# DrQuestion/monica

Hardware: AMD Instinct MI355X
Metric: reads/sec classified (higher is better)
Workload: dtype u32/u64 integer; int16 pairs in the alignment kernels (int32 / int8 in the long-call and literal ones); float32 islands: overlap ratio, MAPQ

## Files before the change

### monica_amd/csrc/k_fill.hip

```cpp
#include "device.h"

namespace mnc {

constexpr int FILL_NEG = -(1 << 28);
constexpr int FILL_WIN = 16;
constexpr int FILL_MIN_BAND = 8;
constexpr int FILL_CIG_MAX = 384;
constexpr size_t FILL_P_SLOT = (size_t)(2 * FILL_MAX_LEN + FILL_WIN) * 64;

__device__ __forceinline__ void fill_order()
{
	__builtin_amdgcn_fence(__ATOMIC_SEQ_CST, "wavefront");
	asm volatile("" ::: "memory");
}
__device__ __forceinline__ void fill_order_mem()
{
	__builtin_amdgcn_fence(__ATOMIC_SEQ_CST, "workgroup");
	asm volatile("" ::: "memory");
}

__device__ __forceinline__ int fill_nt4(uint8_t c)
{
	switch (c) {
	case 'A': case 'a': return 0;
// ... 287 lines not shown
				}
			}
			if (max_zdrop > (B.zdrop_inv < B.zdrop ? B.zdrop_inv : B.zdrop)) to_fb = true;
		}
		const bool s_next = __shfl((int)to_next, lead) != 0, s_fb = __shfl((int)to_fb, lead) != 0;
		const int s_nc = __shfl(n_c, lead);
		if (has && (s_next || s_fb)) {
			if (leader) {
				const bool literal = s_fb || next_list == fb_list;
				if (literal && (B.segs[si].flag & SEG_NEEDS_BIG_WS)) { const unsigned long long k = atomicAdd(&B.dp_ctr[56], 1ULL); B.bigfb_list[k] = (int32_t)si; }
				else if (literal) { const unsigned long long k = atomicAdd(&B.dp_ctr[ctr_fb], 1ULL); fb_list[k] = (int32_t)si; }
				else { const unsigned long long k = atomicAdd(&B.dp_ctr[ctr_next], 1ULL); next_list[k] = (int32_t)si; }
			}
		} else if (has) {
			unsigned long long off = 0;
			if (leader) off = atomicAdd(&B.dp_ctr[1], (unsigned long long)s_nc);
			off = (unsigned long long)__shfl((long long)off, lead);
			int wrote = s_nc;
			if ((long long)(off + s_nc) > B.cig_seg_cap) {
				if (leader) atomicMax(&B.dp_ctr[4], 2ULL);
				wrote = 0;
			} else for (int k = L; k < s_nc; k += LANES) B.cig_seg[off + k] = s_cg[sg][s_nc - 1 - k];
			if (leader) {
				Seg *o = B.segs + si;
				o->n_cigar = wrote, o->zdropped = 0, o->zdrop_code = 0;
				o->max = 0, o->max_t = -1, o->max_q = -1, o->score = S, o->reach_end = 0, o->mqe_t = -1;
				o->cig_off = (int64_t)off;
			}
		}
		fill_order_mem();
	}
}

typedef short pk_s16 __attribute__((ext_vector_type(2)));
typedef unsigned short pk_u16 __attribute__((ext_vector_type(2)));
__device__ __forceinline__ uint32_t pk_adds(uint32_t x, uint32_t y) { return __builtin_bit_cast(uint32_t, __builtin_elementwise_add_sat(__builtin_bit_cast(pk_s16, x), __builtin_bit_cast(pk_s16, y))); }
__device__ __forceinline__ uint32_t pk_subs(uint32_t x, uint32_t y) { return __builtin_bit_cast(uint32_t, __builtin_elementwise_sub_sat(__builtin_bit_cast(pk_s16, x), __builtin_bit_cast(pk_s16, y))); }
__device__ __forceinline__ uint32_t pk_maxs(uint32_t x, uint32_t y) { return __builtin_bit_cast(uint32_t, __builtin_elementwise_max(__builtin_bit_cast(pk_s16, x), __builtin_bit_cast(pk_s16, y))); }
__device__ __forceinline__ uint32_t pk_subsu(uint32_t x, uint32_t y) { return __builtin_bit_cast(uint32_t, __builtin_elementwise_sub_sat(__builtin_bit_cast(pk_u16, x), __builtin_bit_cast(pk_u16, y))); }
__device__ __forceinline__ uint32_t pk_madu(uint32_t x, uint32_t y, uint32_t z) { return __builtin_bit_cast(uint32_t, (pk_u16)(__builtin_bit_cast(pk_u16, x) * __builtin_bit_cast(pk_u16, y) + __builtin_bit_cast(pk_u16, z))); }
__device__ __forceinline__ uint32_t pk_rep(int v) { return ((uint32_t)v & 0xffffu) * 0x10001u; }
__device__ __forceinline__ uint32_t pk_bfi(uint32_t mask, uint32_t x, uint32_t y) { return (x & mask) | (y & ~mask); }

constexpr uint32_t PK_NEG = 0x80008000u;
__device__ __forceinline__ uint32_t fillp_opened(uint32_t x)
{
	const uint32_t d = (x & 1u) ^ 1u, c = (x >> 1 & 1u) ^ d, b = (x >> 2 & 1u) ^ 1u ^ c ^ d, a = (x >> 3 & 1u) ^ b ^ c ^ d;
	return a << 3 | b << 2 | c << 1 | d;
}
constexpr uint32_t PK_TAG_H = 0x000f000fu, PK_TAG_E = 0x00070007u, PK_TAG_F = 0x00030003u, PK_TAG_E2 = 0x00010001u;
struct PkConst { uint32_t kmatch, kmis, q8, q28, e8, e28, de28, dstep; int bias; };

__host__ __device__ __forceinline__ bool fillp_bias(int cells, int a, int bmis_abs, int q, int e, int q2, int e2, int &bias)
{
	const int hi = a * FILL_MAX_LEN, lo = -(bmis_abs * FILL_MAX_LEN + fill_gap(2 * cells + 2, q, e, q2, e2) + (q + e > q2 + e2 ? q + e : q2 + e2));
	bias = -(hi + lo) / 2;
	return hi + bias < 2040 && lo + bias > -2040;
}
__host__ __device__ __forceinline__ bool fillp_drifts(int bmis_abs, int e, int e2) { return bmis_abs == 2 * e && e >= e2; }
__host__ __device__ __forceinline__ bool fillp_bias_drift(int a, int q, int e, int q2, int e2, int &bias)
{
	const int hi = (a + 2 * e) * FILL_MAX_LEN, lo = -(q + e + q2 + e2 + 64);
	bias = -(hi + lo) / 2;
	return hi + bias < 2040 && lo + bias > -2040;
}

template <int K> __device__ __forceinline__ uint32_t fillp_next_q(uint32_t Q2, uint32_t w) { return __builtin_amdgcn_perm(Q2, w, 0x05040c00u + K); }
template <int K> __device__ __forceinline__ uint32_t fillp_next_t(uint32_t T2, uint32_t w) { return __builtin_amdgcn_perm(w, T2, 0x0c040302u + K * 0x10000u); }

#ifndef MNC_FILLP_FRAME2
#define MNC_FILLP_FRAME2 1
#endif
template <int LANES, int ODD, bool EDGE, bool CAPTURE = true, bool DRIFT = false, int KB = -1>
__device__ __forceinline__ void fillp_step(const PkConst &K, const int r, const int L, const int rows_m1, const uint8_t *st, const uint8_t *sq,
                                           const int q, const int e, const int q2, const int e2,
                                           int &t_lo, int &tn, int &jn, uint32_t &T2, uint32_t &Q2, uint32_t &Hs,
                                           uint32_t &E, uint32_t &E2, uint32_t &F, uint32_t &F2, uint32_t &Sc,
                                           uint32_t &nb1, uint32_t &nb2, uint32_t &acc, const uint32_t wq = 0, const uint32_t wt = 0)
{
	constexpr int SHR = LANES == 16 ? 0x111 : 0x138, SHL = LANES == 16 ? 0x101 : 0x130;
	constexpr bool SEG_EDGES = LANES != 16 && LANES != 64;
	uint32_t vE, vE2, vF, vF2;
	if (!ODD) {
		nb1 = (uint32_t)__builtin_amdgcn_update_dpp((int)nb1, (int)E, SHR, 0xf, 0xf, false);
		nb2 = (uint32_t)__builtin_amdgcn_update_dpp((int)nb2, (int)E2, SHR, 0xf, 0xf, false);
		if (SEG_EDGES && L == 0) nb1 = nb2 = PK_NEG;
		vE = __builtin_amdgcn_alignbit(E, nb1, 16), vE2 = __builtin_amdgcn_alignbit(E2, nb2, 16);
		vF = F, vF2 = F2;
		if constexpr (KB >= 0) Q2 = fillp_next_q<KB & 3>(Q2, wq);
		else Q2 = __builtin_amdgcn_perm(Q2, (uint32_t)sq[jn], 0x05040100u), ++jn;
	} else {
		nb1 = (uint32_t)__builtin_amdgcn_update_dpp((int)nb1, (int)F, SHL, 0xf, 0xf, false);
		nb2 = (uint32_t)__builtin_amdgcn_update_dpp((int)nb2, (int)F2, SHL, 0xf, 0xf, false);
		if (SEG_EDGES && L == LANES - 1) nb1 = nb2 = PK_NEG;
		vF = __builtin_amdgcn_alignbit(nb1, F, 16), vF2 = __builtin_amdgcn_alignbit(nb2, F2, 16);
		vE = E, vE2 = E2;
		if constexpr (KB >= 0) T2 = fillp_next_t<KB & 3>(T2, wt);
		else T2 = __builtin_amdgcn_perm((uint32_t)st[tn], T2, 0x05040302u), ++tn;
		if (EDGE) ++t_lo;
	}
	uint32_t hd = Hs;
	if (EDGE) {
		const int hb = -fill_gap(r + 1, q, e, q2, e2) + K.bias + (DRIFT ? e * r : 0);
		const uint32_t h0 = pk_rep(((r == 0 ? 0 : -fill_gap(r, q, e, q2, e2)) + K.bias + (DRIFT ? e * (r - 2) : 0)) << 4) | PK_TAG_H;
		const uint32_t g1 = pk_rep((hb - q - e) << 4), g2 = pk_rep((hb - q2 - e2) << 4);
		const uint32_t mt = t_lo == 0 ? 0x0000ffffu : t_lo == -1 ? 0xffff0000u : 0u;
		const uint32_t mj = t_lo == r ? 0x0000ffffu : t_lo == r - 1 ? 0xffff0000u : 0u;
		hd = pk_bfi(mt | mj, h0, hd);
		vE = pk_bfi(mt, g1 | PK_TAG_E, vE), vE2 = pk_bfi(mt, g2 | PK_TAG_E2, vE2);
		vF = pk_bfi(mj, g1 | PK_TAG_F, vF), vF2 = pk_bfi(mj, g2, vF2);
	}
	uint32_t z;
	if (DRIFT) z = pk_madu(pk_subsu(0x00010001u, T2 ^ Q2), K.kmatch, hd);
	else z = pk_adds(hd, pk_madu(pk_subsu(0x00010001u, T2 ^ Q2), K.kmatch, K.kmis));
	uint32_t o2sub = K.q28;
	constexpr bool FRAME2 = DRIFT && MNC_FILLP_FRAME2 && LANES <= 32;
	if (FRAME2) {
		const uint32_t Dr = (uint32_t)r * K.dstep;
		z = pk_maxs(z, vE), z = pk_maxs(z, vF), z = pk_maxs(z, pk_adds(pk_maxs(vE2, vF2), Dr));
		o2sub = K.q28 + Dr;
	} else z = pk_maxs(z, vE), z = pk_maxs(z, vF), z = pk_maxs(z, vE2), z = pk_maxs(z, vF2);
	const uint32_t zt = z | PK_TAG_H;
	const uint32_t o1 = pk_subs(zt, K.q8), o2 = pk_subs(zt, o2sub);
	const uint32_t mE = pk_maxs(vE, o1), mF = pk_maxs(vF, o1), mE2 = pk_maxs(vE2, o2), mF2 = pk_maxs(vF2, o2);
	if (FRAME2) {
		E = mE & 0xfff7fff7u, F = mF & 0xfff3fff3u, E2 = mE2 & 0xfff1fff1u, F2 = mF2 & 0xfff0fff0u;
	} else if (DRIFT) {
		E = mE & 0xfff7fff7u, F = mF & 0xfff3fff3u;
		E2 = pk_adds(mE2, K.de28) & 0xfff1fff1u, F2 = pk_adds(mF2, K.de28) & 0xfff0fff0u;
	} else {
		E = pk_subs(mE, K.e8) & 0xfff7fff7u;
		F = pk_subs(mF, K.e8) & 0xfff3fff3u;
		E2 = pk_subs(mE2, K.e28) & 0xfff1fff1u;
		F2 = pk_subs(mF2, K.e28) & 0xfff0fff0u;
	}
	const uint32_t x3 = (uint32_t)__builtin_amdgcn_bitop3_b32((int)mE, (int)mF, (int)mE2, 0x96);
	const uint32_t d = pk_bfi(0x000f000fu, z, (x3 ^ mF2) << 4);
	acc = ODD ? __builtin_amdgcn_perm(d, acc, 0x06040200u) : d;
	if (CAPTURE) Sc = r == rows_m1 ? zt : Sc;
	Hs = zt;
}

constexpr int FILLP_G = 16, FILLP_G_MAX = 21;
template <int LANES> struct FillpShape {
	static constexpr int SEGS = 64 / LANES;
	static constexpr int G = SEGS == 3 ? 21 : FILLP_G;
};
constexpr int FILLP_BLOCKS = (2 * FILL_MAX_LEN + 15) / 16 + 1;
constexpr size_t FILLP_PASS_BYTES = (size_t)FILLP_BLOCKS * 64 * 32;
constexpr size_t FILLP_SLOT = FILLP_G_MAX * FILLP_PASS_BYTES;

#ifndef MNC_FILLP_WAVES
#define MNC_FILLP_WAVES 4
#endif
template <int LANES, bool DRIFT>
__global__ __launch_bounds__(64, MNC_FILLP_WAVES) void mnc_dp_fillp(Batch B, const int32_t *list, int ctr_n, int ctr_q, int32_t *next_list, int ctr_next,
                                                   int32_t *fb_list, int ctr_fb, uint8_t *p_all, uint32_t *cig_all)
{
	constexpr int SEGS = FillpShape<LANES>::SEGS, G_MAX = FillpShape<LANES>::G, W = 2 * LANES;
	constexpr int PAD = ((2 * W + 8) & ~7) - 1, SEQ = (FILL_MAX_LEN + 1 + 4 * W + 32 + 7) & ~7;
	static_assert(SEGS * G_MAX <= 64, "one walk per lane");
	constexpr int V = DRIFT ? 1 : 0;
	__shared__ __align__(16) uint8_t s_t[SEGS][SEQ], s_q[SEGS][SEQ];
	__shared__ __align__(16) uint8_t s_chunk[64][32];
	__shared__ int32_t s_n[64], s_m[64], s_kmin[64], s_S[64], s_si[64], s_state[64];
	__shared__ int32_t s_item[64];
	const int lane = threadIdx.x;
	const bool live = lane < SEGS * LANES;
	const int sg = live ? lane / LANES : 0, L = live ? lane % LANES : 0, lead = sg * LANES;
	const bool leader = live && L == 0;
	const int a = B.sc_a, bmis = -B.sc_b, q = B.gap_q, e = B.gap_e, q2 = B.gap_q2, e2 = B.gap_e2;
	PkConst K;
	K.kmatch = pk_rep((DRIFT ? a + 2 * e : a - bmis) << 4), K.kmis = pk_rep(bmis << 4), K.q8 = pk_rep(q << 4), K.q28 = pk_rep(q2 << 4), K.e8 = pk_rep(e << 4), K.e28 = pk_rep(e2 << 4);
	K.de28 = pk_rep((e - e2) << 4), K.dstep = K.de28;
	const bool fits = DRIFT ? fillp_bias_drift(a, q, e, q2, e2, K.bias) : fillp_bias(W, a, -bmis > B.sc_ambi ? -bmis : B.sc_ambi, q, e, q2, e2, K.bias);
	uint8_t *p_wave = p_all + (size_t)blockIdx.x * FILLP_SLOT;
	uint32_t *cg = cig_all + ((size_t)blockIdx.x * 64 + lane) * FILL_CIG_MAX;
	const unsigned long long n_items = B.dp_ctr[ctr_n];
	const unsigned long long segmask = LANES == 64 ? ~0ULL : ((1ULL << (LANES & 63)) - 1) << lead;
	const int thr = B.zdrop_inv < B.zdrop ? B.zdrop_inv : B.zdrop;
	int g_eff = (int)((n_items + (unsigned long long)gridDim.x * SEGS - 1) / ((unsigned long long)gridDim.x * SEGS));
	if (g_eff > G_MAX && g_eff < 2 * G_MAX) g_eff = (g_eff + 1) / 2;
	g_eff = g_eff < 1 ? 1 : g_eff > G_MAX ? G_MAX : g_eff;
	for (;;) {
		unsigned long long q0 = 0;
		if (lane == 0) q0 = atomicAdd(&B.dp_ctr[ctr_q], (unsigned long long)(g_eff * SEGS));
		q0 = (unsigned long long)__shfl((long long)q0, 0);
		if (q0 >= n_items) break;
		s_state[lane] = 0;
		{
			int my_si = -1, my_rows = INT32_MAX;
			if (lane < g_eff * SEGS && q0 + lane < n_items) {
				my_si = list[q0 + lane];
				const Seg *gs = B.segs + my_si;
				my_rows = gs->tlen + gs->qlen;
			}
			int rank = 0;
			for (int j = 0; j < 64; ++j) {
				const int rj = __shfl(my_rows, j);
				rank += (rj < my_rows || (rj == my_rows && j < lane)) ? 1 : 0;
			}
			s_item[rank] = my_si;
		}
		fill_order();
		for (int u = 0; u < g_eff; ++u) {
			if (q0 + (unsigned long long)u * SEGS >= n_items) break;
			const long long si = live ? s_item[u * SEGS + sg] : -1;
			const bool has = si >= 0;
			struct { int32_t tlen, qlen, ts, qs, read, rid, rev; } g = { 0, 0, 0, 0, 0, 0, 0 };
			if (has) {
				const Seg *gs = B.segs + si;
				g.tlen = gs->tlen, g.qlen = gs->qlen, g.ts = gs->ts, g.qs = gs->qs, g.read = gs->read, g.rid = gs->rid, g.rev = gs->rev;
			}
			const int n = g.tlen, m = g.qlen;
			int b, kmin, kmax;
			fill_band(n, m, W, b, kmin, kmax);
			bool ok = has && fits && n >= 1 && m >= 1 && n <= FILL_MAX_LEN && m <= FILL_MAX_LEN && b >= FILL_MIN_BAND;
			bool ambiguous = false;
			if (ok) {
				const uint8_t *read = B.bases + B.offsets[g.read];
				const int rlen = (int)(B.offsets[g.read + 1] - B.offsets[g.read]);
				const int64_t coff = B.seq_off[g.rid] + g.ts;
				const bool acgt = !B.ambig[g.read];
				const int64_t roff = B.offsets[g.read];
				if (V) {
					const uint32_t sh = (uint32_t)(coff & 7) * 4;
#pragma unroll 1
					for (int i = 8 * L; i < n; i += 8 * LANES) {
						const bool more = sh != 0 && i + 8 - (int)(coff & 7) < n;
						const uint32_t a0 = B.seq4[((coff + i) >> 3)], a1 = more ? B.seq4[((coff + i) >> 3) + 1] : 0u;
						const uint32_t v = sh ? __builtin_amdgcn_alignbit(a1, a0, sh) : a0;
						ambiguous |= (v & 0xccccccccu & (n - i < 8 ? (1u << (4 * (n - i))) - 1u : ~0u)) != 0;
						uint2 w;
						w.x = v & 0xffffu, w.x = (w.x | w.x << 8) & 0x00ff00ffu, w.x = (w.x | w.x << 4) & 0x03030303u;
						w.y = v >> 16, w.y = (w.y | w.y << 8) & 0x00ff00ffu, w.y = (w.y | w.y << 4) & 0x03030303u;
						*reinterpret_cast<uint2*>(&s_t[sg][PAD + 1 + i]) = w;
					}
					if (acgt) {
#pragma unroll 1
						for (int i = 16 * L; i < m; i += 16 * LANES) {
							const uint32_t f = fill_qcodes16(B, roff, rlen, g.rev, g.qs + i);
							uint32_t x[4];
#pragma unroll
							for (int k = 0; k < 4; ++k) {
								const uint32_t b8 = f >> (8 * k) & 0xffu;
								x[k] = (b8 | b8 << 12) & 0x000f000fu, x[k] = (x[k] | x[k] << 6) & 0x03030303u;
							}
							*reinterpret_cast<uint2*>(&s_q[sg][PAD + 1 + i]) = make_uint2(x[0], x[1]);
							*reinterpret_cast<uint2*>(&s_q[sg][PAD + 1 + i + 8]) = make_uint2(x[2], x[3]);
						}
					} else {
#pragma unroll 1
						for (int i = L; i < m; i += LANES) {
							const int c = fill_qcode(B, false, roff, read, rlen, g.rev, g.qs + i);
							ambiguous |= c > 3;
							s_q[sg][PAD + 1 + i] = (uint8_t)(c & 3);
						}
					}
					if (L == 0) s_t[sg][PAD] = 4, s_q[sg][PAD] = 5;
				} else {
#pragma unroll 1
					for (int i = L; i < n; i += LANES) {
						const int64_t o = coff + i;
						const uint32_t c = B.seq4[o >> 3] >> ((o & 7) * 4) & 15u;
						ambiguous |= c > 3;
						s_t[sg][PAD + i] = (uint8_t)(c & 3);
					}
#pragma unroll 1
					for (int i = L; i < m; i += LANES) {
						const int c = fill_qcode(B, acgt, roff, read, rlen, g.rev, g.qs + i);
						ambiguous |= c > 3;
						s_q[sg][PAD + i] = (uint8_t)(c & 3);
					}
				}
			}
			const bool seg_amb = (__ballot(ambiguous && live) & segmask) != 0;
			const bool to_fb = ok && seg_amb;
			ok = ok && !seg_amb;
			fill_order();
			const int rows = ok ? n + m - 1 + 2 * V : 0;
			int max_rows = (rows + 15) & ~15, edge_rows = ok && !V ? ((-kmin > kmax ? -kmin : kmax) + 2 + 15) & ~15 : 0;
			{
				int mr = 0, er = 0;
#pragma unroll
				for (int s2 = 0; s2 < SEGS; ++s2) {
					const int o = __builtin_amdgcn_readlane(max_rows, s2 * LANES), oe = __builtin_amdgcn_readlane(edge_rows, s2 * LANES);
					mr = mr > o ? mr : o, er = er > oe ? er : oe;
				}
				max_rows = mr, edge_rows = er;
			}
			int cap_from = ok ? (rows - 1) & ~15 : INT32_MAX;
			{
				int cf = INT32_MAX;
#pragma unroll
				for (int s2 = 0; s2 < SEGS; ++s2) { const int o = __builtin_amdgcn_readlane(cap_from, s2 * LANES); cf = cf < o ? cf : o; }
				cap_from = cf < max_rows ? cf : max_rows;
			}
			if (edge_rows > max_rows) edge_rows = max_rows;
			const int kmin_run = ok ? kmin : -2 * W;
			const uint8_t *st = &s_t[sg][0], *sq = &s_q[sg][0];
			int t_lo = (kmin_run >> 1) + 2 * L;
			uint32_t T2 = (uint32_t)st[PAD + t_lo] | (uint32_t)st[PAD + t_lo + 1] << 16;
			uint32_t Q2 = (uint32_t)sq[PAD - t_lo - 1] | (uint32_t)sq[PAD - t_lo - 2] << 16;
			int tn = PAD + t_lo + 2, jn = PAD - t_lo;
			uint32_t He = PK_NEG | PK_TAG_H, Ho = He, E = PK_NEG | PK_TAG_E, F = PK_NEG | PK_TAG_F, E2 = PK_NEG | PK_TAG_E2, F2 = PK_NEG, Sc = PK_NEG;
			uint32_t nbe1 = PK_NEG, nbe2 = PK_NEG, nbf1 = PK_NEG, nbf2 = PK_NEG;
			if (V && ok) {
				const int cc = -kmin >> 1;
				if (L == cc >> 1) He = pk_bfi(cc & 1 ? 0xffff0000u : 0x0000ffffu, pk_rep(K.bias << 4) | PK_TAG_H, He);
			}
			const int rows_m1 = rows - 1;
			uint4 *pblk = reinterpret_cast<uint4*>(p_wave + (size_t)u * FILLP_PASS_BYTES + lane * 32);
			int r = 0;
			for (; r < edge_rows; r += 16, pblk += 2048 / 16) {
				uint32_t acc[8];
#pragma unroll
				for (int k = 0; k < 8; ++k) {
					fillp_step<LANES, 0, true, true, DRIFT>(K, r + 2 * k, L, rows_m1, st, sq, q, e, q2, e2, t_lo, tn, jn, T2, Q2, He, E, E2, F, F2, Sc, nbe1, nbe2, acc[k]);
					fillp_step<LANES, 1, true, true, DRIFT>(K, r + 2 * k + 1, L, rows_m1, st, sq, q, e, q2, e2, t_lo, tn, jn, T2, Q2, Ho, E, E2, F, F2, Sc, nbf1, nbf2, acc[k]);
				}
				pblk[0] = make_uint4(acc[0], acc[1], acc[2], acc[3]), pblk[1] = make_uint4(acc[4], acc[5], acc[6], acc[7]);
			}
#define MNC_FILLP_PAIR(CAP, k) \
	fillp_step<LANES, 0, false, CAP, DRIFT, k>(K, r + 2 * k, L, rows_m1, st, sq, q, e, q2, e2, t_lo, tn, jn, T2, Q2, He, E, E2, F, F2, Sc, nbe1, nbe2, acc[k], k < 4 ? wq.x : wq.y, 0u); \
	fillp_step<LANES, 1, false, CAP, DRIFT, k>(K, r + 2 * k + 1, L, rows_m1, st, sq, q, e, q2, e2, t_lo, tn, jn, T2, Q2, Ho, E, E2, F, F2, Sc, nbf1, nbf2, acc[k], 0u, k < 4 ? wt.x : wt.y);
#define MNC_FILLP_BLOCK(CAP) { \
	uint32_t acc[8]; \
	uint2 wq, wt; \
	__builtin_memcpy(&wq, sq + jn, 8), __builtin_memcpy(&wt, st + tn, 8); \
	jn += 8, tn += 8; \
	MNC_FILLP_PAIR(CAP, 0) MNC_FILLP_PAIR(CAP, 1) MNC_FILLP_PAIR(CAP, 2) MNC_FILLP_PAIR(CAP, 3) \
	MNC_FILLP_PAIR(CAP, 4) MNC_FILLP_PAIR(CAP, 5) MNC_FILLP_PAIR(CAP, 6) MNC_FILLP_PAIR(CAP, 7) \
	pblk[0] = make_uint4(acc[0], acc[1], acc[2], acc[3]), pblk[1] = make_uint4(acc[4], acc[5], acc[6], acc[7]); }
			for (; r < cap_from; r += 16, pblk += 2048 / 16) MNC_FILLP_BLOCK(false)
			for (; r < max_rows; r += 16, pblk += 2048 / 16) MNC_FILLP_BLOCK(true)
#undef MNC_FILLP_BLOCK
#undef MNC_FILLP_PAIR
			int S = FILL_NEG;
			{
				int lc = ok ? n - 1 + V - ((rows - 1 + kmin + 1) >> 1) : 0;
				lc = lc < 0 ? 0 : lc >= W ? W - 1 : lc;
				const uint32_t v = (uint32_t)__shfl((int)Sc, lead + (lc >> 1));
				S = ((int)(int16_t)(lc & 1 ? v >> 16 : v & 0xffffu) >> 4) - K.bias - (DRIFT ? e * (rows - 1) : 0);
				const int U = dp_band_bound(n, m, kmin, kmax, a, q, e, q2, e2);
				if (ok && !(S > U)) ok = false;
			}
			if (leader && has) {
				const int w = u * SEGS + sg;
				s_n[w] = n + V, s_m[w] = m + V, s_kmin[w] = kmin, s_S[w] = S, s_si[w] = (int32_t)si;
				s_state[w] = ok ? 1 : to_fb ? 3 : 2;
			}
			fill_order();
		}
		fill_order_mem();
		int state_w = lane < g_eff * SEGS ? s_state[lane] : 0;
		const int n = s_n[lane], m = s_m[lane], kmin = s_kmin[lane], S = s_S[lane];
		const long long si = s_si[lane];
		int n_c = 0;
		{
			const uint8_t *pu = p_wave + (size_t)(lane / SEGS) * FILLP_PASS_BYTES + (lane % SEGS) * LANES * 32;
			int bi = n - 1, bj = m - 1, state = 0, cid = -1, mcols = 0, g2 = 0, kd = 0, kbest = 0;
			uint32_t cur = 0, hm32 = 0;
			bool walking = state_w == 1;
			while (walking && bi >= V && bj >= V) {
				const int r = bi + bj, idx = bi - ((r + kmin + 1) >> 1);
				if (idx < 0 || idx >= W) { state_w = 2; walking = false; break; }
				const int c = (r >> 4) * 64 + (idx >> 1);
				if (c != cid) {
					const uint4 *src = reinterpret_cast<const uint4*>(pu + (size_t)c * 32);
					const uint4 v0 = src[0], v1 = src[1];
					*reinterpret_cast<uint4*>(&s_chunk[lane][0]) = v0, *reinterpret_cast<uint4*>(&s_chunk[lane][16]) = v1;
					cid = c;
					const uint32_t w8[8] = { v0.x, v0.y, v0.z, v0.w, v1.x, v1.y, v1.z, v1.w };
					hm32 = 0;
#pragma unroll
					for (int k = 0; k < 8; ++k) hm32 |= (w8[k] >> 3 & 0x01010101u) << k;
				}
				if (state == 0) {
					const int rho = r & 15, bp = rho >> 1;
					const uint32_t m8 = hm32 >> (8 * ((rho & 1) * 2 + (idx & 1))) & 0xffu;
					const uint32_t zeros = ~m8 & ((2u << bp) - 1u);
					int run = zeros ? bp - (31 - __clz((int)zeros)) : bp + 1;
					const int lim = (bi < bj ? bi : bj) + 1 - V;
					run = run < lim ? run : lim;
					if (run > 0) {
						if (cur != 0 && (cur & 0xf) == 0) cur += (uint32_t)run << 4;
						else {
							if (cur != 0) {
								if (n_c >= FILL_CIG_MAX - 4) { state_w = 3; walking = false; break; }
								const int len = (int)(cur >> 4);
								g2 += fill_gap(len, q, e, q2, e2), kd += q + e * len, kbest = kbest > kd ? kbest : kd;
								cg[n_c++] = cur;
							}
							cur = (uint32_t)run << 4;
						}
						bi -= run, bj -= run;
						continue;
					}
				}
				const uint32_t raw = s_chunk[lane][(r & 15) * 2 + (idx & 1)];
				if (state != 0 && (fillp_opened(raw >> 4) >> (4 - state) & 1u)) state = 0;
				if (state == 0) { const uint32_t tag = raw & 15u; state = tag >= 8u ? 0 : tag == 7u ? 1 : tag == 3u ? 2 : tag == 1u ? 3 : 4; }
				uint32_t op;
				if (state == 0) op = 0, --bi, --bj;
				else if (state == 1 || state == 3) op = 2, --bi;
				else op = 1, --bj;
				if (cur != 0 && (cur & 0xf) == op) cur += 1u << 4;
				else {
					if (cur != 0) {
						if (n_c >= FILL_CIG_MAX - 4) { state_w = 3; walking = false; break; }
						const int len = (int)(cur >> 4);
						if ((cur & 0xf) == 0) mcols += len, kd = kd - a * len > 0 ? kd - a * len : 0;
						else g2 += fill_gap(len, q, e, q2, e2), kd += q + e * len, kbest = kbest > kd ? kbest : kd;
						cg[n_c++] = cur;
					}
					cur = 1u << 4 | op;
				}
			}
			if (walking) {
				auto push = [&](uint32_t w) {
					const int len = (int)(w >> 4);
					if ((w & 0xf) == 0) mcols += len, kd = kd - a * len > 0 ? kd - a * len : 0;
					else g2 += fill_gap(len, q, e, q2, e2), kd += q + e * len, kbest = kbest > kd ? kbest : kd;
					cg[n_c++] = w;
				};
				if (bi >= V) { if (cur != 0 && (cur & 0xf) == 2) cur += (uint32_t)(bi + 1 - V) << 4; else { if (cur != 0) push(cur); cur = (uint32_t)(bi + 1 - V) << 4 | 2; } }
				if (bj >= V) { if (cur != 0 && (cur & 0xf) == 1) cur += (uint32_t)(bj + 1 - V) << 4; else { if (cur != 0) push(cur); cur = (uint32_t)(bj + 1 - V) << 4 | 1; } }
				if (cur != 0) push(cur);
				const int lost = a * mcols - S - g2;
				const int neg = kbest + lost;
				if (neg > thr) state_w = 4;
			}
		}
		fill_order_mem();
		if (state_w == 4) {
			const Seg *gs = B.segs + si;
			const uint8_t *read = B.bases + B.offsets[gs->read];
			const int rlen = (int)(B.offsets[gs->read + 1] - B.offsets[gs->read]), rev = gs->rev, qs = gs->qs;
			const int64_t coff = B.seq_off[gs->rid] + gs->ts;
			int score = 0, mx = INT32_MIN, max_i = -1, max_j = -1, i = 0, j = 0, max_zdrop = 0;
			for (int k = n_c - 1; k >= 0; --k) {
				const uint32_t w = cg[k], op = w & 0xf;
				const int len = (int)(w >> 4);
				if (op == 0) {
					for (int l = 0; l < len; ++l) {
						const int64_t o = coff + i + l;
						const int ct = (int)(B.seq4[o >> 3] >> ((o & 7) * 4) & 15u), pq = qs + j + l;
						int cq = fill_nt4(read[rev ? rlen - 1 - pq : pq]);
						if (rev) cq = 3 - cq;
						score += ct == cq ? a : bmis;
						if (score < mx) {
							const int li = i + l - max_i, lj = j + l - max_j;
							const int z = mx - score - (li > lj ? li - lj : lj - li) * e;
							max_zdrop = max_zdrop > z ? max_zdrop : z;
						} else mx = score, max_i = i + l, max_j = j + l;
					}
					i += len, j += len;
				} else {
					score -= q + e * len;
					if (op == 1) j += len; else i += len;
					if (score < mx) {
						const int li = i - max_i, lj = j - max_j;
						const int z = mx - score - (li > lj ? li - lj : lj - li) * e;
						max_zdrop = max_zdrop > z ? max_zdrop : z;
					} else mx = score, max_i = i, max_j = j;
				}
			}
			state_w = max_zdrop > thr ? 3 : 1;
		}
		if (state_w == 2) { const unsigned long long k = atomicAdd(&B.dp_ctr[ctr_next], 1ULL); next_list[k] = (int32_t)si; }
		if (state_w == 3) { const unsigned long long k = atomicAdd(&B.dp_ctr[ctr_fb], 1ULL); fb_list[k] = (int32_t)si; }
		{
			const int mine = state_w == 1 ? n_c : 0;
			int incl = mine;
#pragma unroll
			for (int sft = 1; sft < 64; sft <<= 1) { const int o = __shfl_up(incl, sft); if (lane >= sft) incl += o; }
			const int total = __shfl(incl, 63);
			unsigned long long base = 0;
			if (lane == 0 && total > 0) base = atomicAdd(&B.dp_ctr[1], (unsigned long long)total);
			base = (unsigned long long)__shfl((long long)base, 0);
			if ((long long)(base + total) > B.cig_seg_cap) {
				if (lane == 0) atomicMax(&B.dp_ctr[4], 2ULL);
				if (state_w == 1) { Seg *o = B.segs + si; o->n_cigar = 0, o->zdropped = 0, o->zdrop_code = 0, o->cig_off = 0; }
			} else if (state_w == 1) {
				const unsigned long long off = base + (unsigned long long)(incl - mine);
				for (int k = 0; k < n_c; ++k) B.cig_seg[off + k] = cg[n_c - 1 - k];
				Seg *o = B.segs + si;
				o->n_cigar = n_c, o->zdropped = 0, o->zdrop_code = 0;
				o->max = 0, o->max_t = -1, o->max_q = -1, o->score = S, o->reach_end = 0, o->mqe_t = -1;
				o->cig_off = (int64_t)off;
			}
		}
		fill_order_mem();
	}
}

template <int LANES, int CPL, int MAXLEN>
__global__ __launch_bounds__(64) void mnc_dp_ext(Batch B, const int32_t *list, int ctr_n, int ctr_q, int32_t *fb_list, int ctr_fb, uint8_t *p_all)
{
	constexpr int SEGS = 64 / LANES, W = LANES * CPL, ROWB = 64 * CPL, SEQ = 2 * MAXLEN + 2;
	static_assert(CPL == 1 || LANES == 64, "several cells per lane: one segment per wave");
	__shared__ uint8_t s_t[SEGS][SEQ], s_q[SEGS][SEQ];
	__shared__ __align__(16) uint8_t s_win[SEGS][FILL_WIN * W];
	__shared__ uint32_t s_cg[SEGS][SEQ];
	const int lane = threadIdx.x, sg = lane / LANES, L = lane % LANES, lead = sg * LANES;
	const bool leader = L == 0;
	const int a = B.sc_a, bmis = -B.sc_b, scN = -B.sc_ambi, q = B.gap_q, e = B.gap_e, q2 = B.gap_q2, e2 = B.gap_e2;
	uint8_t *p_wave = p_all + (size_t)blockIdx.x * ((size_t)(2 * MAXLEN + FILL_WIN) * 64 * CPL);
	const unsigned long long n_items = B.dp_ctr[ctr_n];
	if (MAXLEN > FILL_MAX_LEN) __builtin_amdgcn_s_setprio(3);
	for (;;) {
		unsigned long long q0 = 0;
		if (lane == 0) q0 = atomicAdd(&B.dp_ctr[ctr_q], (unsigned long long)SEGS);
		q0 = (unsigned long long)__shfl((long long)q0, 0);
		if (q0 >= n_items) break;
		const bool has = q0 + sg < n_items;
		const long long si = has ? (long long)list[q0 + sg] : -1;
		struct { int32_t tlen, qlen, ts, qs, read, rid, rev, kind, zdrop, flag; } g = { 0, 0, 0, 0, 0, 0, 0, 0, 0, 0 };
		if (has) {
			const Seg *gs = B.segs + si;
			g.tlen = gs->tlen, g.qlen = gs->qlen, g.ts = gs->ts, g.qs = gs->qs, g.read = gs->read, g.rid = gs->rid, g.rev = gs->rev;
			g.kind = gs->kind, g.zdrop = gs->zdrop, g.flag = gs->flag;
		}
		const int n = g.tlen, m = g.qlen;
		const int mn = n < m ? n : m;
		const bool ok = has && n >= 1 && m >= 1 && mn <= W && n + m - 1 <= 2 * MAXLEN;
		const int rgt = (g.flag & EZ_RIGHT) ? 1 : 0;
		if (ok) {
			const uint8_t *read = B.bases + B.offsets[g.read];
			const int rlen = (int)(B.offsets[g.read + 1] - B.offsets[g.read]);
			const int64_t coff = B.seq_off[g.rid];
			const bool rv = g.kind == 0;
			for (int i = L; i < n; i += LANES) {
				const int64_t o = coff + (rv ? g.ts + n - 1 - i : g.ts + i);
				s_t[sg][i] = (uint8_t)(B.seq4[o >> 3] >> ((o & 7) * 4) & 15u);
			}
			const bool acgt = !B.ambig[g.read];
			const int64_t roff = B.offsets[g.read];
			for (int i = L; i < m; i += LANES) s_q[sg][i] = (uint8_t)fill_qcode(B, acgt, roff, read, rlen, g.rev, rv ? g.qs + m - 1 - i : g.qs + i);
		}
		fill_order();
		const int rows = ok ? n + m - 1 : 0;
		int max_rows = rows;
		if (SEGS == 2) { const int o = __shfl_xor(max_rows, 32); max_rows = max_rows > o ? max_rows : o; }
		int ez_max = 0, ez_max_t = -1, ez_max_q = -1, ez_mqe = DP_NEG_INF, ez_mqe_t = -1, zdropped = 0;
		int H1[CPL], H2[CPL], En[CPL], E2n[CPL], Fn[CPL], F2n[CPL];
#pragma unroll
		for (int k = 0; k < CPL; ++k) H1[k] = H2[k] = En[k] = E2n[k] = Fn[k] = F2n[k] = FILL_NEG;
		uint8_t *prow = p_wave + lead * CPL + L;
		int done = 0;
		for (int r = 0; r < max_rows; ++r, prow += ROWB) {
			if (__all(zdropped || done || r >= rows)) break;
			const int st0 = r - m + 1 > 0 ? r - m + 1 : 0, en0 = r < n - 1 ? r : n - 1;
			const int en1 = st0 + (en0 - st0) / 4 * 4;
			unsigned long long key = 0;
			int h_first = FILL_NEG;
			int sE_[CPL], sE2_[CPL], sF_[CPL], sF2_[CPL], hd_[CPL];
#pragma unroll
			for (int k = 0; k < CPL; ++k) {
				int uE = __builtin_amdgcn_update_dpp(FILL_NEG, En[k], 0x138, 0xf, 0xf, false), uE2 = __builtin_amdgcn_update_dpp(FILL_NEG, E2n[k], 0x138, 0xf, 0xf, false);
				int uH = __builtin_amdgcn_update_dpp(FILL_NEG, H2[k], 0x138, 0xf, 0xf, false);
				int dF = __builtin_amdgcn_update_dpp(FILL_NEG, Fn[k], 0x130, 0xf, 0xf, false), dF2 = __builtin_amdgcn_update_dpp(FILL_NEG, F2n[k], 0x130, 0xf, 0xf, false);
				int dH = __builtin_amdgcn_update_dpp(FILL_NEG, H2[k], 0x130, 0xf, 0xf, false);
				if (L == 0) {
					if (k == 0) uE = uE2 = uH = FILL_NEG;
					else uE = __builtin_amdgcn_readlane(En[k > 0 ? k - 1 : 0], 63), uE2 = __builtin_amdgcn_readlane(E2n[k > 0 ? k - 1 : 0], 63), uH = __builtin_amdgcn_readlane(H2[k > 0 ? k - 1 : 0], 63);
				}
				if (L == LANES - 1) {
					if (k == CPL - 1) dF = dF2 = dH = FILL_NEG;
					else dF = __builtin_amdgcn_readlane(Fn[k + 1 < CPL ? k + 1 : k], 0), dF2 = __builtin_amdgcn_readlane(F2n[k + 1 < CPL ? k + 1 : k], 0), dH = __builtin_amdgcn_readlane(H2[k + 1 < CPL ? k + 1 : k], 0);
				}
				sE_[k] = r < m ? uE : En[k], sE2_[k] = r < m ? uE2 : E2n[k];
				sF_[k] = r < m ? Fn[k] : dF, sF2_[k] = r < m ? F2n[k] : dF2;
				hd_[k] = r < m ? uH : r == m ? H2[k] : dH;
			}
#pragma unroll
			for (int k = 0; k < CPL; ++k) {
				int sE = sE_[k], sE2 = sE2_[k], sF = sF_[k], sF2 = sF2_[k], hd = hd_[k];
				const int t = st0 + L + LANES * k, j = r - t;
				const bool act = !zdropped && !done && r < rows && t <= en0;
				int Hn = FILL_NEG, nEn = FILL_NEG, nE2n = FILL_NEG, nFn = FILL_NEG, nF2n = FILL_NEG;
				if (act) {
					const int ct = s_t[sg][t], cq = s_q[sg][j];
					const int sc = (ct == 4 || cq == 4) ? scN : ct == cq ? a : bmis;
					if (t == 0 || j == 0) {
						hd = t == 0 && j == 0 ? 0 : -fill_gap(t == 0 ? j : t, q, e, q2, e2);
						if (t == 0) { const int hb = -fill_gap(j + 1, q, e, q2, e2); sE = hb - q - e, sE2 = hb - q2 - e2; }
// ... 445 lines not shown
				if (ok) ez_mqe = (pk_half(bq, cm & 1) >> 4) - K.bias, ez_mqe_t = (int)((cm & 1) ? bqr >> 16 : bqr & 0xffffu) - cm;
			}
			if (leader && has) {
				const int w = u * SEGS + sg;
				int bi = -1, bj = -1, reach_end = 0;
				if (ok && !suspect) {
					if (ez_mqe + B.end_bonus > ez_max) reach_end = 1, bi = ez_mqe_t, bj = m - 1;
					else if (ez_max_t >= 0 && ez_max_q >= 0) bi = ez_max_t, bj = ez_max_q;
				}
				s_n[w] = n, s_m[w] = m, s_bi[w] = bi, s_bj[w] = bj, s_si[w] = (int32_t)si, s_keep[w] = (g.flag & EZ_REV_CIGAR) != 0;
				s_max[w] = ez_max, s_maxt[w] = ez_max_t, s_maxq[w] = ez_max_q, s_mqet[w] = ez_mqe_t, s_reach[w] = reach_end;
				s_state[w] = ok && !suspect ? 1 : 2;
			}
			fill_order();
		}
		fill_order_mem();
		int state_w = lane < g_eff * SEGS ? s_state[lane] : 0;
		const int n = s_n[lane], m = s_m[lane];
		const long long si = s_si[lane];
		int n_c = 0;
		if (state_w == 1) {
			const uint8_t *pu = p_wave + (size_t)(lane / SEGS) * PASS_BYTES;
			const int slot = lane % SEGS;
			int bi = s_bi[lane], bj = s_bj[lane], state = 0, cid = -1;
			uint32_t cur = 0;
			bool walking = bi >= 0 && bj >= 0, bad = false;
			while (walking && bi >= 0 && bj >= 0) {
				const int r = bi + bj;
				const int c = ((r >> 4) * 64 + slot * LANES + bj / (2 * CPL)) * CPL + bj % (2 * CPL) / 2;
				if (c != cid) {
					const uint4 *src = reinterpret_cast<const uint4*>(pu + (size_t)c * 32);
					const uint4 v0 = src[0], v1 = src[1];
					*reinterpret_cast<uint4*>(&s_chunk[lane][0]) = v0, *reinterpret_cast<uint4*>(&s_chunk[lane][16]) = v1;
					cid = c;
				}
				const uint32_t raw = s_chunk[lane][(r & 15) * 2 + (bj & 1)], tag = raw & 15u;
				if (RGT) {
					if (state != 0 && !(extp_extended(raw >> 4) >> (state - 1) & 1u)) state = 0;
					if (state == 0) state = tag == 0u ? 0 : tag == 1u ? 1 : tag == 3u ? 2 : tag == 7u ? 3 : 4;
				} else {
					if (state != 0 && (fillp_opened(raw >> 4) >> (4 - state) & 1u)) state = 0;
					if (state == 0) state = tag >= 8u ? 0 : tag == 7u ? 1 : tag == 3u ? 2 : tag == 1u ? 3 : 4;
				}
				uint32_t op;
				if (state == 0) op = 0, --bi, --bj;
				else if (state == 1 || state == 3) op = 2, --bi;
				else op = 1, --bj;
				if (cur != 0 && (cur & 0xf) == op) cur += 1u << 4;
				else {
					if (cur != 0) {
						if (n_c >= EXTP_CIG_MAX - 4) { bad = true; break; }
						cg[n_c++] = cur;
					}
					cur = 1u << 4 | op;
				}
			}
			if (bad) state_w = 2;
			else if (walking) {
				if (bi >= 0) { if (cur != 0 && (cur & 0xf) == 2) cur += (uint32_t)(bi + 1) << 4; else { if (cur != 0) cg[n_c++] = cur; cur = (uint32_t)(bi + 1) << 4 | 2; } }
				if (bj >= 0) { if (cur != 0 && (cur & 0xf) == 1) cur += (uint32_t)(bj + 1) << 4; else { if (cur != 0) cg[n_c++] = cur; cur = (uint32_t)(bj + 1) << 4 | 1; } }
				if (cur != 0) cg[n_c++] = cur;
			}
		}
		fill_order_mem();
		if (state_w == 2) {
			const int mn = n < m ? n : m;
			const int ci = mn <= 32 ? 16 : mn <= 64 ? 17 : mn <= 128 ? 24 : 25;
			int32_t *lst = mn <= 32 ? B.ext_list1 : mn <= 64 ? B.ext_list2 : mn <= 128 ? B.ext_list3 : B.ext_list4;
			if (mn <= 256) { const unsigned long long k = atomicAdd(&B.dp_ctr[ci], 1ULL); lst[k] = (int32_t)si; }
			else { const unsigned long long k = atomicAdd(&B.dp_ctr[12], 1ULL); B.fill_fb[k] = (int32_t)si; }
		}
		{
			const int mine = state_w == 1 ? n_c : 0;
			int incl = mine;
#pragma unroll
			for (int sft = 1; sft < 64; sft <<= 1) { const int o = __shfl_up(incl, sft); if (lane >= sft) incl += o; }
			const int total = __shfl(incl, 63);
			unsigned long long base = 0;
			if (lane == 0 && total > 0) base = atomicAdd(&B.dp_ctr[1], (unsigned long long)total);
			base = (unsigned long long)__shfl((long long)base, 0);
			const bool over = (long long)(base + total) > B.cig_seg_cap;
			if (over && lane == 0) atomicMax(&B.dp_ctr[4], 2ULL);
			if (state_w == 1) {
				const unsigned long long off = base + (unsigned long long)(incl - mine);
				const bool keep = s_keep[lane] != 0;
				if (!over) for (int k = 0; k < n_c; ++k) B.cig_seg[off + k] = cg[keep ? k : n_c - 1 - k];
				Seg *o = B.segs + si;
				o->n_cigar = over ? 0 : n_c, o->zdropped = 0, o->zdrop_code = 0;
				o->max = s_max[lane], o->max_t = s_maxt[lane], o->max_q = s_maxq[lane], o->score = DP_NEG_INF, o->reach_end = s_reach[lane], o->mqe_t = s_mqet[lane];
				o->cig_off = (int64_t)off;
			}
		}
		fill_order_mem();
	}
}

size_t dp_extp_slot() { return (size_t)EXTP_G * FILLP_BLOCKS * 64 * 32 * 2; }
size_t dp_extp_cig_slot() { return (size_t)64 * EXTP_CIG_MAX * 4; }
void launch_dp_extp(const Batch &B, int cells, int rgt, const int32_t *list, int ctr_n, int ctr_q, uint8_t *p_all, uint32_t *cig_all, int n_wg, hipStream_t st)
{
#define MNC_EXTP(LN, CP) do { if (rgt) hipLaunchKernelGGL((mnc_dp_extp<LN, CP, 1>), dim3(n_wg), dim3(64), 0, st, B, list, ctr_n, ctr_q, p_all, cig_all); \
	else hipLaunchKernelGGL((mnc_dp_extp<LN, CP, 0>), dim3(n_wg), dim3(64), 0, st, B, list, ctr_n, ctr_q, p_all, cig_all); } while (0)
	if (cells == 32) MNC_EXTP(16, 1);
	else if (cells == 64) MNC_EXTP(32, 1);
	else if (cells == 128) MNC_EXTP(64, 1);
	else MNC_EXTP(64, 2);
#undef MNC_EXTP
}

constexpr int LFILL_MAX_LEN = 2047, LFILL_CIG_MAX = 1024;
size_t dp_lfill_p_slot() { return (size_t)(2 * LFILL_MAX_LEN + FILL_WIN) * 64 * 4; }
void launch_dp_lfill(const Batch &B, const int32_t *list, int ctr_n, int ctr_q, int32_t *fb_list, int ctr_fb, uint8_t *p_all, int n_wg, hipStream_t st)
{
	hipLaunchKernelGGL((mnc_dp_fill<64, 4, LFILL_MAX_LEN, LFILL_CIG_MAX>), dim3(n_wg), dim3(64), 0, st, B, list, ctr_n, ctr_q, fb_list, ctr_fb, fb_list, ctr_fb, p_all);
}
constexpr int LEXT_MAX_LEN = 1535;
size_t dp_lext_p_slot() { return (size_t)(2 * LEXT_MAX_LEN + FILL_WIN) * 64 * 8; }
void launch_dp_lext(const Batch &B, const int32_t *list, int ctr_n, int ctr_q, int32_t *fb_list, int ctr_fb, uint8_t *p_all, int n_wg, hipStream_t st)
{
	hipLaunchKernelGGL((mnc_dp_ext<64, 8, LEXT_MAX_LEN>), dim3(n_wg), dim3(64), 0, st, B, list, ctr_n, ctr_q, fb_list, ctr_fb, p_all);
}
size_t dp_fill_p_slot() { return FILL_P_SLOT; }
size_t dp_fillp_slot() { return FILLP_SLOT; }
size_t dp_fillp_cig_slot() { return (size_t)64 * FILL_CIG_MAX * 4; }
void launch_dp_fill(const Batch &B, int lanes, const int32_t *list, int ctr_n, int ctr_q, int32_t *next_list, int ctr_next,
                    int32_t *fb_list, int ctr_fb, uint8_t *p_all, uint32_t *cig_all, int n_wg, hipStream_t st)
{
	bool drift = fillp_drifts(B.sc_b, B.gap_e, B.gap_e2) && !(B.debug_route & 1024);
	if (drift && MNC_FILLP_FRAME2 && lanes <= 64) {
		int bias = 0;
		const bool fits = fillp_bias_drift(B.sc_a, B.gap_q, B.gap_e, B.gap_q2, B.gap_e2, bias);
		const int floor_pts = 2048 + bias;
		const int qmax = B.gap_q > B.gap_q2 ? B.gap_q : B.gap_q2, emax = B.gap_e > B.gap_e2 ? B.gap_e : B.gap_e2;
		const int need = B.sc_a * (lanes + 1) + 2 * qmax + emax * 2 * (lanes + 1) + (B.gap_q2 + B.gap_e2) + 16;
		if (!fits || need >= floor_pts) drift = false;
	}
#define MNC_LAUNCH_FILLP(LN) do { if (drift) hipLaunchKernelGGL((mnc_dp_fillp<LN, true>), dim3(n_wg), dim3(64), 0, st, B, list, ctr_n, ctr_q, next_list, ctr_next, fb_list, ctr_fb, p_all, cig_all); \
	else hipLaunchKernelGGL((mnc_dp_fillp<LN, false>), dim3(n_wg), dim3(64), 0, st, B, list, ctr_n, ctr_q, next_list, ctr_next, fb_list, ctr_fb, p_all, cig_all); } while (0)
	if (lanes == 32) MNC_LAUNCH_FILLP(16);
	else if (lanes == FILL_MID_CELLS) MNC_LAUNCH_FILLP(FILL_MID_CELLS / 2);
	else if (lanes == 64) MNC_LAUNCH_FILLP(32);
	else MNC_LAUNCH_FILLP(64);
#undef MNC_LAUNCH_FILLP
}

void launch_dp_ext(const Batch &B, int lanes, const int32_t *list, int ctr_n, int ctr_q, int32_t *fb_list, int ctr_fb, uint8_t *p_all, int n_wg, hipStream_t st)
{
	if (lanes == 32) hipLaunchKernelGGL((mnc_dp_ext<32, 1, FILL_MAX_LEN>), dim3(n_wg), dim3(64), 0, st, B, list, ctr_n, ctr_q, fb_list, ctr_fb, p_all);
	else if (lanes == 64) hipLaunchKernelGGL((mnc_dp_ext<64, 1, FILL_MAX_LEN>), dim3(n_wg), dim3(64), 0, st, B, list, ctr_n, ctr_q, fb_list, ctr_fb, p_all);
	else if (lanes == 128) hipLaunchKernelGGL((mnc_dp_ext<64, 2, FILL_MAX_LEN>), dim3(n_wg), dim3(64), 0, st, B, list, ctr_n, ctr_q, fb_list, ctr_fb, p_all);
	else hipLaunchKernelGGL((mnc_dp_ext<64, 4, FILL_MAX_LEN>), dim3(n_wg), dim3(64), 0, st, B, list, ctr_n, ctr_q, fb_list, ctr_fb, p_all);
}

}
```

Measured before the change: 2.915 million.

## Shrink fill tail to 4-row granularity and keep traceback run-skips on-chunk

The fill kernel's capture tail now pads rows to a multiple of 4 instead of 16. It runs an unrolled-once loop of 4 rows per step that loads 2 bytes of sequence and writes half-words into the pointer block. This cuts the wasted DP rows past the true end of each segment. The traceback no longer restarts the loop after a diagonal run when it can continue in place, and the hm32 bit extraction is rewritten with per-k shifts. Optional atomic counters behind MNC_FILLP_COUNT are added for profiling. The smaller tail loop trades the 16-row unroll's amortisation for fewer rows computed.

```diff
diff --git a/monica_amd/csrc/k_fill.hip b/monica_amd/csrc/k_fill.hip
--- a/monica_amd/csrc/k_fill.hip
+++ b/monica_amd/csrc/k_fill.hip
@@ -463,6 +463,10 @@
 
 #ifndef MNC_FILLP_WAVES
 #define MNC_FILLP_WAVES 4
+#endif
+#ifdef MNC_FILLP_COUNT
+__device__ unsigned long long g_fillp_count[4][16];
+#define MNC_FILLP_CNT(k, v) atomicAdd(&g_fillp_count[LANES == 16 ? 0 : LANES == 32 ? 2 : LANES == 64 ? 3 : 1][k], (unsigned long long)(v))
 #endif
 template <int LANES, bool DRIFT>
 __global__ __launch_bounds__(64, MNC_FILLP_WAVES) void mnc_dp_fillp(Batch B, const int32_t *list, int ctr_n, int ctr_q, int32_t *next_list, int ctr_next,
@@ -590,7 +594,7 @@
 			ok = ok && !seg_amb;
 			fill_order();
 			const int rows = ok ? n + m - 1 + 2 * V : 0;
-			int max_rows = (rows + 15) & ~15, edge_rows = ok && !V ? ((-kmin > kmax ? -kmin : kmax) + 2 + 15) & ~15 : 0;
+			int max_rows = (rows + 3) & ~3, edge_rows = ok && !V ? ((-kmin > kmax ? -kmin : kmax) + 2 + 15) & ~15 : 0;
 			{
 				int mr = 0, er = 0;
 #pragma unroll
@@ -607,7 +611,7 @@
 				for (int s2 = 0; s2 < SEGS; ++s2) { const int o = __builtin_amdgcn_readlane(cap_from, s2 * LANES); cf = cf < o ? cf : o; }
 				cap_from = cf < max_rows ? cf : max_rows;
 			}
-			if (edge_rows > max_rows) edge_rows = max_rows;
+			if (edge_rows > ((max_rows + 15) & ~15)) edge_rows = (max_rows + 15) & ~15;
 			const int kmin_run = ok ? kmin : -2 * W;
 			const uint8_t *st = &s_t[sg][0], *sq = &s_q[sg][0];
 			int t_lo = (kmin_run >> 1) + 2 * L;
@@ -632,21 +636,43 @@
 				}
 				pblk[0] = make_uint4(acc[0], acc[1], acc[2], acc[3]), pblk[1] = make_uint4(acc[4], acc[5], acc[6], acc[7]);
 			}
-#define MNC_FILLP_PAIR(CAP, k) \
-	fillp_step<LANES, 0, false, CAP, DRIFT, k>(K, r + 2 * k, L, rows_m1, st, sq, q, e, q2, e2, t_lo, tn, jn, T2, Q2, He, E, E2, F, F2, Sc, nbe1, nbe2, acc[k], k < 4 ? wq.x : wq.y, 0u); \
-	fillp_step<LANES, 1, false, CAP, DRIFT, k>(K, r + 2 * k + 1, L, rows_m1, st, sq, q, e, q2, e2, t_lo, tn, jn, T2, Q2, Ho, E, E2, F, F2, Sc, nbf1, nbf2, acc[k], 0u, k < 4 ? wt.x : wt.y);
+#define MNC_FILLP_PAIR(CAP, k, WQ, WT) \
+	fillp_step<LANES, 0, false, CAP, DRIFT, k>(K, r + 2 * k, L, rows_m1, st, sq, q, e, q2, e2, t_lo, tn, jn, T2, Q2, He, E, E2, F, F2, Sc, nbe1, nbe2, acc[k], WQ, 0u); \
+	fillp_step<LANES, 1, false, CAP, DRIFT, k>(K, r + 2 * k + 1, L, rows_m1, st, sq, q, e, q2, e2, t_lo, tn, jn, T2, Q2, Ho, E, E2, F, F2, Sc, nbf1, nbf2, acc[k], 0u, WT);
 #define MNC_FILLP_BLOCK(CAP) { \
 	uint32_t acc[8]; \
 	uint2 wq, wt; \
 	__builtin_memcpy(&wq, sq + jn, 8), __builtin_memcpy(&wt, st + tn, 8); \
 	jn += 8, tn += 8; \
-	MNC_FILLP_PAIR(CAP, 0) MNC_FILLP_PAIR(CAP, 1) MNC_FILLP_PAIR(CAP, 2) MNC_FILLP_PAIR(CAP, 3) \
-	MNC_FILLP_PAIR(CAP, 4) MNC_FILLP_PAIR(CAP, 5) MNC_FILLP_PAIR(CAP, 6) MNC_FILLP_PAIR(CAP, 7) \
+	MNC_FILLP_PAIR(CAP, 0, wq.x, wt.x) MNC_FILLP_PAIR(CAP, 1, wq.x, wt.x) MNC_FILLP_PAIR(CAP, 2, wq.x, wt.x) MNC_FILLP_PAIR(CAP, 3, wq.x, wt.x) \
+	MNC_FILLP_PAIR(CAP, 4, wq.y, wt.y) MNC_FILLP_PAIR(CAP, 5, wq.y, wt.y) MNC_FILLP_PAIR(CAP, 6, wq.y, wt.y) MNC_FILLP_PAIR(CAP, 7, wq.y, wt.y) \
 	pblk[0] = make_uint4(acc[0], acc[1], acc[2], acc[3]), pblk[1] = make_uint4(acc[4], acc[5], acc[6], acc[7]); }
 			for (; r < cap_from; r += 16, pblk += 2048 / 16) MNC_FILLP_BLOCK(false)
-			for (; r < max_rows; r += 16, pblk += 2048 / 16) MNC_FILLP_BLOCK(true)
+#ifdef MNC_FILLP_COUNT
+			if (lane == 0) MNC_FILLP_CNT(3, max_rows > r ? max_rows - r : 0);
+#endif
+#pragma unroll 1
+			for (; r < max_rows; r += 4) {
+				uint32_t acc[2];
+				uint16_t hq, ht;
+				__builtin_memcpy(&hq, sq + jn, 2), __builtin_memcpy(&ht, st + tn, 2);
+				jn += 2, tn += 2;
+				const uint32_t wq = hq, wt = ht;
+				MNC_FILLP_PAIR(true, 0, wq, wt) MNC_FILLP_PAIR(true, 1, wq, wt)
+				*reinterpret_cast<uint2*>(reinterpret_cast<uint8_t*>(pblk) + (r & 12) * 2) = make_uint2(acc[0], acc[1]);
+				if ((r & 12) == 12) pblk += 2048 / 16;
+			}
 #undef MNC_FILLP_BLOCK
 #undef MNC_FILLP_PAIR
+#ifdef MNC_FILLP_COUNT
+			if (lane == 0) MNC_FILLP_CNT(1, 1), MNC_FILLP_CNT(2, r), MNC_FILLP_CNT(12, (r + 15) & ~15);
+			if (leader && ok) MNC_FILLP_CNT(11, rows);
+			{
+				int lt = ok ? (n + 8 * LANES - 1) / (8 * LANES) : 0, lq = ok ? (m + 16 * LANES - 1) / (16 * LANES) : 0, mt = 0, mq = 0;
+				for (int s2 = 0; s2 < SEGS; ++s2) { const int o = __shfl(lt, s2 * LANES), p = __shfl(lq, s2 * LANES); mt = mt > o ? mt : o, mq = mq > p ? mq : p; }
+				if (lane == 0) MNC_FILLP_CNT(8, mt), MNC_FILLP_CNT(9, mq);
+			}
+#endif
 			int S = FILL_NEG;
 			{
 				int lc = ok ? n - 1 + V - ((rows - 1 + kmin + 1) >> 1) : 0;
@@ -667,6 +693,9 @@
 		int state_w = lane < g_eff * SEGS ? s_state[lane] : 0;
 		const int n = s_n[lane], m = s_m[lane], kmin = s_kmin[lane], S = s_S[lane];
 		const long long si = s_si[lane];
+#ifdef MNC_FILLP_COUNT
+		int cnt_turns = 0, cnt_loads = 0, cnt_same = 0;
+#endif
 		int n_c = 0;
 		{
 			const uint8_t *pu = p_wave + (size_t)(lane / SEGS) * FILLP_PASS_BYTES + (lane % SEGS) * LANES * 32;
@@ -674,9 +703,13 @@
 			uint32_t cur = 0, hm32 = 0;
 			bool walking = state_w == 1;
 			while (walking && bi >= V && bj >= V) {
-				const int r = bi + bj, idx = bi - ((r + kmin + 1) >> 1);
+				int r = bi + bj;
+				const int idx = bi - ((r + kmin + 1) >> 1);
 				if (idx < 0 || idx >= W) { state_w = 2; walking = false; break; }
 				const int c = (r >> 4) * 64 + (idx >> 1);
+#ifdef MNC_FILLP_COUNT
+				++cnt_turns, cnt_loads += c != cid ? 1 : 0;
+#endif
 				if (c != cid) {
 					const uint4 *src = reinterpret_cast<const uint4*>(pu + (size_t)c * 32);
 					const uint4 v0 = src[0], v1 = src[1];
@@ -685,7 +718,7 @@
 					const uint32_t w8[8] = { v0.x, v0.y, v0.z, v0.w, v1.x, v1.y, v1.z, v1.w };
 					hm32 = 0;
 #pragma unroll
-					for (int k = 0; k < 8; ++k) hm32 |= (w8[k] >> 3 & 0x01010101u) << k;
+					for (int k = 0; k < 8; ++k) hm32 |= (k < 3 ? w8[k] >> (3 - k) : w8[k] << (k - 3)) & (0x01010101u << k);
 				}
 				if (state == 0) {
 					const int rho = r & 15, bp = rho >> 1;
@@ -706,7 +739,11 @@
 							cur = (uint32_t)run << 4;
 						}
 						bi -= run, bj -= run;
-						continue;
+						if (zeros == 0 || bi < V || bj < V) continue;
+						r -= 2 * run;
+#ifdef MNC_FILLP_COUNT
+						++cnt_same;
+#endif
 					}
 				}
 				const uint32_t raw = s_chunk[lane][(r & 15) * 2 + (idx & 1)];
@@ -744,6 +781,18 @@
 			}
 		}
 		fill_order_mem();
+#ifdef MNC_FILLP_COUNT
+		{
+			int mt = 0, mc = 0, mo = 0;
+			for (int j = 0; j < 64; ++j) {
+				const int o = __shfl(cnt_turns, j), p = __shfl(state_w == 1 || state_w == 4 ? n_c : 0, j), o2 = __shfl(cnt_turns + cnt_same, j);
+				mt = mt > o ? mt : o, mc = mc > p ? mc : p, mo = mo > o2 ? mo : o2;
+			}
+			MNC_FILLP_CNT(5, cnt_turns), MNC_FILLP_CNT(6, cnt_loads);
+			if (lane == 0) MNC_FILLP_CNT(0, 1), MNC_FILLP_CNT(4, mt), MNC_FILLP_CNT(7, mc), MNC_FILLP_CNT(13, mo);
+			if (__any(state_w == 4) && lane == 0) MNC_FILLP_CNT(10, 1);
+		}
+#endif
 		if (state_w == 4) {
 			const Seg *gs = B.segs + si;
 			const uint8_t *read = B.bases + B.offsets[gs->read];
@@ -1495,4 +1544,16 @@
 	else hipLaunchKernelGGL((mnc_dp_ext<64, 4, FILL_MAX_LEN>), dim3(n_wg), dim3(64), 0, st, B, list, ctr_n, ctr_q, fb_list, ctr_fb, p_all);
 }
 
-}
+
+#ifdef MNC_FILLP_COUNT
+}
+extern "C" int mnc_debug_fillp_counts(long long *out64, int reset)
+{
+	unsigned long long z[64] = {0};
+	if (out64 && hipMemcpyFromSymbol(out64, HIP_SYMBOL(mnc::g_fillp_count), sizeof(z)) != hipSuccess) return -1;
+	if (reset && hipMemcpyToSymbol(HIP_SYMBOL(mnc::g_fillp_count), z, sizeof(z)) != hipSuccess) return -1;
+	return 0;
+}
+namespace mnc {
+#endif
+}
```

After: 2.931 million (median of 6 runs). No clear change (+0.6%).
